# vovach777/llcomp

Measured on AMD Instinct MI355X. Metric: encode+decode MPix/s on 4K RGB8, bit-exact, higher is better.
Workload: dtype int32

## Files before the change

### llcomp_amd/csrc/codec.hip

```cpp
#include <hip/hip_runtime.h>

#include <algorithm>
#include <cstdlib>
#include <cstring>
#include <mutex>
#include <new>
#include <vector>

#include "../../include/llcomp_mi.h"
#include "codec_internal.hpp"
#include "container.hpp"
#include "geometry.hpp"
#include "kernels.hpp"
#include "resize.hpp"
#include "snapshot.hpp"
#include "tables.hpp"

using namespace llcomp_mi;

namespace llcomp_mi {

int status_from_bits(uint32_t bits) {
    if (bits & kStInternal) return LLCOMP_MI_HIP_ERROR;
    if (bits & kStBadExponent) return LLCOMP_MI_BAD_EXPONENT;
// ... 604 lines not shown
                    dev_alloc(reinterpret_cast<void**>(&k->d_scratch), b_scratch) == hipSuccess &&
                    dev_alloc(reinterpret_cast<void**>(&k->d_group_off), b_off) == hipSuccess &&
                    dev_alloc(reinterpret_cast<void**>(&k->d_total_tmp), 8) == hipSuccess &&
                    dev_alloc(reinterpret_cast<void**>(&k->d_counters), kCtrCount * 8) == hipSuccess &&
                    hipMemset(k->d_counters, 0, kCtrCount * 8) == hipSuccess;
    if (!ok) {
        llcomp_mi_codec_destroy(k);
        return LLCOMP_MI_NOMEM;
    }
    k->allocated_bytes = b_sym + b_lanes + b_scratch + b_off + 8;
    *out = k;
    return LLCOMP_MI_OK;
}

extern "C" {

void llcomp_mi_codec_destroy(llcomp_mi_codec* k) {
    llcomp_mi::codec_release(k);
}

int llcomp_mi_codec_prepare(llcomp_mi_codec* k, uint32_t what) {
    if (!k || (what & ~(LLCOMP_MI_PREPARE_ENCODE | LLCOMP_MI_PREPARE_DECODE | LLCOMP_MI_PREPARE_REGION | LLCOMP_MI_PREPARE_REGIONS |
                        LLCOMP_MI_PREPARE_RESIZED)))
        return LLCOMP_MI_BAD_ARGS;
    DeviceGuard guard(k->device);
    if (!guard.ok) return LLCOMP_MI_HIP_ERROR;
    if (what & LLCOMP_MI_PREPARE_ENCODE) {
        if (snapshot_mode(k->g)) {
            if (int rc = ensure_snapshot_arrays(k)) return rc;
        }
        if (!snapshot_mode(k->g) || snapshot_chunked(k->g))
            if (int rc = ensure_state_tables(k, k->need_states)) return rc;
    }
    if (what & LLCOMP_MI_PREPARE_DECODE)
        if (int rc = ensure_state_tables(k, k->need_states)) return rc;
    if (what & (LLCOMP_MI_PREPARE_REGION | LLCOMP_MI_PREPARE_REGIONS | LLCOMP_MI_PREPARE_RESIZED)) {
        if (int rc = ensure_region_arrays(k)) return rc;
        if (region_may_need_states(k))
            if (int rc = ensure_state_tables(k, true)) return rc;
    }
    if (what & LLCOMP_MI_PREPARE_REGIONS)
        if (int rc = ensure_regions_table(k)) return rc;
    if (what & LLCOMP_MI_PREPARE_RESIZED) {
        const uint64_t samples = uint64_t(k->g.frames) * k->g.w * k->g.h * k->g.c;
        if (int rc = ensure_regions_ring(k)) return rc;
        if (int rc = ensure_grown(k, k->d_box, k->box_cap, samples, samples)) return rc;
        if (int rc = ensure_grown(k, k->d_mid, k->mid_cap, samples, samples)) return rc;
    }
    return LLCOMP_MI_OK;
}

uint32_t llcomp_mi_codec_slices(const llcomp_mi_codec* k) { return k ? k->g.n_slices : 0; }
uint32_t llcomp_mi_codec_kernel_family(const llcomp_mi_codec* k) { return k ? (k->g.flags & 0xFFu) | (k->g.lane_shift << 8) | (k->g.lpw << 16) : 0; }
uint64_t llcomp_mi_codec_workspace_bytes(const llcomp_mi_codec* k) { return k ? k->workspace_bytes : 0; }
uint64_t llcomp_mi_codec_allocated_bytes(const llcomp_mi_codec* k) { return k ? k->allocated_bytes : 0; }
uint64_t llcomp_mi_codec_max_payload_bytes(const llcomp_mi_codec* k) {
    return k ? uint64_t(k->g.n_slices) * k->g.slice_cap : 0;
}

int llcomp_mi_codec_model(llcomp_mi_codec* k, const void* d_px, void* d_sym, void* stream) {
    if (!k || !d_px || !d_sym) return LLCOMP_MI_BAD_ARGS;
    DeviceGuard guard(k->device);
    if (!guard.ok) return LLCOMP_MI_HIP_ERROR;
    HIP_TRY(launch_model_fwd(k->g, static_cast<const uint8_t*>(d_px), static_cast<uint32_t*>(d_sym),
                             static_cast<hipStream_t>(stream)));
    return LLCOMP_MI_OK;
}

int llcomp_mi_codec_encode(llcomp_mi_codec* k, const void* d_px, void* d_payload, uint64_t payload_cap, void* d_slice_len,
                           void* d_total, void* d_status, void* stream) {
    if (!k || !d_px || !d_payload || !d_slice_len || !d_total || !d_status) return LLCOMP_MI_BAD_ARGS;
    DeviceGuard guard(k->device);
    if (!guard.ok) return LLCOMP_MI_HIP_ERROR;
    hipStream_t s = static_cast<hipStream_t>(stream);
    const Geometry& g = k->g;
    DoneGuard done_guard{k, s};
    HIP_TRY(hipMemsetAsync(d_status, 0, 4, s));
    if (!snapshot_mode(g) || snapshot_chunked(g)) {
        Timed t(k, s, 0);
        if (int rc = next_state_generation(k, s, k->need_states)) return rc;
    }
    {
        Timed t(k, s, 1);
        if (model_is_fused(g)) {
            HIP_TRY(launch_model_rows_fwd(g, static_cast<const uint8_t*>(d_px), static_cast<uint16_t*>(k->d_lane_order), s));
        } else {
            HIP_TRY(launch_model_fwd(g, static_cast<const uint8_t*>(d_px), static_cast<uint32_t*>(k->d_sym_or_rec), s));
            if (!snapshot_mode(g))
                HIP_TRY(launch_to_lane_order_u32(g, static_cast<const uint32_t*>(k->d_sym_or_rec),
                                                 static_cast<uint32_t*>(k->d_lane_order), s));
        }
    }
    if (snapshot_mode(g) && snapshot_chunked(g)) {
        if (int rc = ensure_snapshot_arrays(k)) return rc;
        const uint64_t gpat = state_generation_tag(k->state_generation);
        const uint32_t chunks = snapshot_chunks(g);
        hipStream_t ps = k->overlap ? k->aux : s;
        if (k->overlap) {
            HIP_TRY(hipEventRecord(k->ev_fork, s));
            HIP_TRY(hipStreamWaitEvent(k->aux, k->ev_fork, 0));
        }
        auto pass = [&](uint32_t c) -> int {
            Timed t(k, ps, 0);
            HIP_TRY(launch_snapshot_chunk(g, c, static_cast<const uint32_t*>(k->d_sym_or_rec), k->d_lane_order, k->d_snap_sorted, k->d_snap_banks,
                                          k->d_snap_res, k->d_snap_ctx, k->d_snap_io, k->d_states, gpat, ps));
            return LLCOMP_MI_OK;
        };
        auto coder = [&](uint32_t c) -> int {
            Timed t(k, s, 2);
            HIP_TRY(launch_encode_segment(g, k->d_snap_res, static_cast<uint64_t*>(k->d_snap_banks), k->d_scratch, static_cast<uint32_t*>(d_slice_len),
                                          static_cast<uint32_t*>(d_status), k->d_counters, c * kSnapMaxSamples, k->d_seg_state, s));
            return LLCOMP_MI_OK;
        };
        int rc = LLCOMP_MI_OK;
        if (k->overlap) {
            for (uint32_t c = 0; c < chunks && !rc; ++c) {
                rc = pass(c);
                if (!rc && hipEventRecord(k->ev_chunk[c], k->aux) != hipSuccess) rc = LLCOMP_MI_HIP_ERROR;
            }
            for (uint32_t c = 0; c < chunks; ++c) {
                if (hipStreamWaitEvent(s, k->ev_chunk[c], 0) != hipSuccess) { (void)hipGetLastError(); (void)hipStreamSynchronize(k->aux); }
                if (!rc) rc = coder(c);
            }
        } else {
            for (uint32_t c = 0; c < chunks && !rc; ++c) {
                rc = pass(c);
                if (!rc) rc = coder(c);
            }
        }
        if (rc) return rc;
    } else {
    if (snapshot_mode(g)) {
        if (int rc = ensure_snapshot_arrays(k)) return rc;
        Timed t(k, s, 0);
        HIP_TRY(launch_snapshot(g, static_cast<const uint32_t*>(k->d_sym_or_rec), k->d_lane_order, k->d_snap_sorted,
                                k->d_snap_banks, k->d_snap_res, s));
    }
    {
        Timed t(k, s, 2);
        const bool snap = snapshot_mode(g);
        HIP_TRY(launch_encode_slices(g, snap ? k->d_snap_res : k->d_lane_order, snap ? static_cast<uint64_t*>(k->d_snap_banks) : k->d_states,
                                     k->state_generation, k->d_scratch, static_cast<uint32_t*>(d_slice_len),
                                     k->d_group_off, static_cast<uint32_t*>(d_status), k->d_counters, s));
    }
    }
    {
        Timed t(k, s, 3);
        if (!encoder_writes_group_sums(g)) HIP_TRY(launch_group_sums(g, static_cast<const uint32_t*>(d_slice_len), k->d_group_off, s));
        HIP_TRY(launch_scan_groups(g, k->d_group_off, static_cast<uint64_t*>(d_total), s));
        HIP_TRY(launch_pack_payload(g, k->d_scratch, static_cast<const uint32_t*>(d_slice_len), k->d_group_off,
                                    static_cast<uint8_t*>(d_payload), payload_cap, static_cast<uint32_t*>(d_status), s));
    }
    ++k->n_encode;
    return LLCOMP_MI_OK;
}

int llcomp_mi_codec_decode(llcomp_mi_codec* k, const void* d_payload, uint64_t payload_bytes, const void* d_slice_len,
                           void* d_px, void* d_status, void* stream) {
    if (!k || !d_payload || !d_slice_len || !d_px || !d_status) return LLCOMP_MI_BAD_ARGS;
    DeviceGuard guard(k->device);
    if (!guard.ok) return LLCOMP_MI_HIP_ERROR;
    hipStream_t s = static_cast<hipStream_t>(stream);
    const Geometry& g = k->g;
    DoneGuard done_guard{k, s};
    HIP_TRY(hipMemsetAsync(d_status, 0, 4, s));
    {
        Timed t(k, s, 7);
        if (int rc = next_state_generation(k, s, k->need_states)) return rc;
    }
    {
        Timed t(k, s, 4);
        HIP_TRY(launch_group_sums(g, static_cast<const uint32_t*>(d_slice_len), k->d_group_off, s));
        HIP_TRY(launch_scan_groups(g, k->d_group_off, k->d_total_tmp, s));
    }
    {
        Timed t(k, s, 4);
        HIP_TRY(launch_stage_streams(g, static_cast<const uint8_t*>(d_payload), payload_bytes,
                                     static_cast<const uint32_t*>(d_slice_len), k->d_group_off, k->d_scratch,
                                     static_cast<uint32_t*>(d_status), s));
    }
    {
        Timed t(k, s, 5);
        const bool cache = use_bank_cache(k, g);
        HIP_TRY(launch_decode_slices(g, k->d_scratch, static_cast<const uint32_t*>(d_slice_len), k->d_states, k->state_generation,
                                     static_cast<int16_t*>(k->d_lane_order), static_cast<uint32_t*>(d_status), k->d_counters, cache, s));
        if (cache) queue_feedback(k, s);
    }
    {
        Timed t(k, s, 6);
        if (model_is_fused(g)) {
            HIP_TRY(launch_model_rows_inv(g, static_cast<const int16_t*>(k->d_lane_order), static_cast<uint8_t*>(d_px), s));
        } else {
            HIP_TRY(launch_from_lane_order_i16(g, static_cast<const int16_t*>(k->d_lane_order),
                                               static_cast<int16_t*>(k->d_sym_or_rec), s));
            HIP_TRY(launch_model_inv(g, static_cast<const int16_t*>(k->d_sym_or_rec), static_cast<uint8_t*>(d_px), s));
        }
    }
    ++k->n_decode;
    return LLCOMP_MI_OK;
}

uint32_t llcomp_mi_codec_region_family(const llcomp_mi_codec* k, uint32_t x, uint32_t y, uint32_t rw, uint32_t rh) {
    RegionBox box;
    Geometry sub;
    if (!k || region_setup(k, x, y, rw, rh, box, sub)) return 0;
    return (sub.flags & 0xFFu) | (sub.lane_shift << 8) | (sub.lpw << 16);
}

int llcomp_mi_codec_decode_region(llcomp_mi_codec* k, const void* d_payload, uint64_t payload_bytes, const void* d_slice_len, uint32_t x,
                                  uint32_t y, uint32_t rw, uint32_t rh, void* d_px, void* d_status, void* stream) {
    if (!k || !d_payload || !d_slice_len || !d_px || !d_status) return LLCOMP_MI_BAD_ARGS;
    RegionBox box;
    Geometry sub;
    if (int rc = region_setup(k, x, y, rw, rh, box, sub)) return rc;
    DeviceGuard guard(k->device);
    if (!guard.ok) return LLCOMP_MI_HIP_ERROR;
    if (int rc = ensure_region_arrays(k)) return rc;
    hipStream_t s = static_cast<hipStream_t>(stream);
    const Geometry& g = k->g;
    DoneGuard done_guard{k, s};
    HIP_TRY(hipMemsetAsync(d_status, 0, 4, s));
    {
        Timed t(k, s, 7);
        if (int rc = next_state_generation(k, s, slices_need_state_tables(sub))) return rc;
// ... 298 lines not shown
```

### llcomp_amd/csrc/geometry.hpp

```cpp
#pragma once
#include <algorithm>
#include <cstdint>
#include <cstdlib>

#if defined(__HIPCC__)
#define LLMI_HD __host__ __device__
#else
#define LLMI_HD
#endif

namespace llcomp_mi {

constexpr uint32_t kMaxChannels = 255;

struct Geometry {
    uint32_t frames, w, h, c;
    uint32_t tile_w, tile_h, planar;
    uint32_t ntx, nty;
    uint32_t slices_per_frame;
    uint32_t n_slices;
    uint32_t slice_cap;
    uint32_t nch;
    uint32_t lane_shift;
    uint32_t slice_samples;
    uint32_t lpw;
    uint32_t flags;
};
enum : uint32_t {
    kGeoRows = 1u,
    kGeoLdsTable = 2u,
    kGeoForceReplay = 4u,
    kGeoSmallModel = 8u,
    kGeoSnapshot = 16u,
    kGeoBankCache = 32u,
};
constexpr uint32_t kSnapMaxSamples = 4096;
constexpr uint32_t kSnapMaxChunks = 4;

struct Tuning {
    int lane_shift = -1;
    int lpw = 0;
    bool norows = false;
    bool noldstab = false;
    bool force_replay = false;
    bool nosnap = false;
    bool nocache = false;
    int overlap = 2;
    bool nofeedback = false;
};
inline Tuning tuning_from_env() {
    Tuning t;
    auto num = [](const char* name, long lo, long hi, int dflt) {
        const char* e = std::getenv(name);
        if (!e || !*e) return dflt;
        const long v = std::strtol(e, nullptr, 10);
        return (v >= lo && v <= hi) ? int(v) : dflt;
    };
    auto flag = [](const char* name) { const char* e = std::getenv(name); return e && e[0] == '1'; };
    t.lane_shift = num("LLCOMP_MI_LANE_SHIFT", 0, 6, -1);
    t.lpw = num("LLCOMP_MI_LPW", 1, 64, 0);
    t.norows = flag("LLCOMP_MI_NOROWS");
    t.noldstab = flag("LLCOMP_MI_NOLDSTAB");
    t.force_replay = flag("LLCOMP_MI_FORCE_REPLAY");
    t.nosnap = flag("LLCOMP_MI_NOSNAP");
    t.nocache = flag("LLCOMP_MI_NOCACHE");
    t.nofeedback = flag("LLCOMP_MI_NOFEEDBACK");
    t.overlap = num("LLCOMP_MI_OVERLAP", 0, 2, 2);
    return t;
}

LLMI_HD inline uint32_t snapshot_chunks(const Geometry& g) { return (g.slice_samples + kSnapMaxSamples - 1) / kSnapMaxSamples; }
LLMI_HD inline uint32_t snapshot_cap(const Geometry& g) {
    return g.slice_samples <= kSnapMaxSamples ? (g.slice_samples + 15u) & ~15u : snapshot_chunks(g) * kSnapMaxSamples;
}

constexpr int kBankCacheLog2 = 5;
inline int bank_cache_log2(const Geometry& g) { return (g.flags & kGeoBankCache) ? kBankCacheLog2 : 0; }

LLMI_HD inline size_t lane_order_index(const Geometry& g, uint32_t id, uint32_t k) {
    const uint32_t gw = 1u << g.lane_shift;
    return ((size_t(id >> g.lane_shift) * g.slice_samples + k) << g.lane_shift) + (id & (gw - 1));
}

struct SliceRect {
    uint32_t frame, x0, y0, sw, sh, ch;
};

LLMI_HD inline SliceRect slice_rect(const Geometry& g, uint32_t id) {
    SliceRect r;
    r.frame = id / g.slices_per_frame;
    uint32_t s = id - r.frame * g.slices_per_frame;
    uint32_t tile = s;
    r.ch = 0;
    if (g.planar) {
        tile = s / g.c;
        r.ch = s - tile * g.c;
    }
    const uint32_t ty = tile / g.ntx, tx = tile - ty * g.ntx;
    r.x0 = tx * g.tile_w;
    r.y0 = ty * g.tile_h;
    r.sw = g.w - r.x0 < g.tile_w ? g.w - r.x0 : g.tile_w;
    r.sh = g.h - r.y0 < g.tile_h ? g.h - r.y0 : g.tile_h;
    return r;
}

inline uint32_t default_lane_shift(uint32_t n_slices) {
    constexpr uint32_t kMinWaves = 96;
    uint32_t s = 6;
    while (s > 0 && (n_slices >> s) < kMinWaves) --s;
    return s;
}

inline bool make_geometry(Geometry& g, uint32_t frames, uint32_t w, uint32_t h, uint32_t c, uint32_t tile_w,
                          uint32_t tile_h, uint32_t planar, const Tuning& tune = Tuning{}, bool small_model = false) {
    if (!frames || !w || !h || c < 1 || c > kMaxChannels) return false;
    if (tile_w == 0 || tile_w > w) tile_w = w;
    if (tile_h == 0 || tile_h > h) tile_h = h;
    const uint64_t samples = uint64_t(w) * h * c;
    if (samples >= (1ull << 31)) return false;
    g.frames = frames; g.w = w; g.h = h; g.c = c;
    g.tile_w = tile_w; g.tile_h = tile_h; g.planar = planar ? 1 : 0;
    g.ntx = (w + tile_w - 1) / tile_w;
    g.nty = (h + tile_h - 1) / tile_h;
    const uint64_t spf = uint64_t(g.ntx) * g.nty * (g.planar ? c : 1);
    if (spf * frames >= (1ull << 31)) return false;
    g.slices_per_frame = uint32_t(spf);
    g.n_slices = uint32_t(spf * frames);
    g.nch = g.planar ? 1 : c;
    const uint64_t cap = (uint64_t(tile_w) * tile_h * g.nch * 13 + 32 + 15) & ~15ull;
    g.slice_cap = uint32_t(cap < 0x7FFFFFF0ull ? cap : 0x7FFFFFF0ull);
    g.slice_samples = tile_w * tile_h * g.nch;
    g.lane_shift = tune.lane_shift >= 0 ? uint32_t(tune.lane_shift) : default_lane_shift(g.n_slices);
    if (tune.lane_shift < 0 && g.tile_h > 1 && g.slice_samples > kSnapMaxSamples && g.n_slices <= 512) g.lane_shift = 0;
    const uint32_t gw = 1u << g.lane_shift;
    g.lpw = gw;
    if (tune.lpw >= 1) {
        uint32_t p = 1;
        while (p * 2 <= uint32_t(tune.lpw) && p * 2 <= gw) p *= 2;
        g.lpw = p;
    }
    g.flags = 0;
    if (g.tile_h == 1 && !tune.norows && g.nch <= 4) g.flags |= kGeoRows;
    else if (g.lpw == 1 && !tune.noldstab) g.flags |= kGeoLdsTable;
    else if (g.slice_samples <= kSnapMaxSamples * kSnapMaxChunks && !tune.nosnap) g.flags |= kGeoSnapshot;
    if (!(g.flags & (kGeoRows | kGeoLdsTable)) && g.nch <= 4 && !tune.nocache) g.flags |= kGeoBankCache;
    if (tune.force_replay) g.flags |= kGeoForceReplay;
    if (small_model) g.flags |= kGeoSmallModel;
    return true;
}

inline uint64_t legacy_read_bound(uint64_t samples) { return 65 * samples + 2; }
inline void fit_legacy_stream(Geometry& g, uint64_t bytes) {
    const uint64_t cap = (bytes + 16 + 15) & ~15ull;
    if (cap > g.slice_cap) g.slice_cap = uint32_t(cap < 0x7FFFFFF0ull ? cap : 0x7FFFFFF0ull);
}

struct RegionBox {
    uint32_t tx0, ty0, tx1, ty1;
};
inline bool region_box(uint32_t w, uint32_t h, uint32_t tile_w, uint32_t tile_h, uint32_t x, uint32_t y, uint32_t rw, uint32_t rh,
// ... 85 lines not shown
```

### llcomp_amd/csrc/kernels.hpp

```cpp
#pragma once
#include <hip/hip_runtime.h>

#include <cstdint>

#include "geometry.hpp"

namespace llcomp_mi {

enum : uint32_t { kStOverflow = 1u, kStBadExponent = 2u, kStTruncated = 4u, kStInternal = 8u  };

enum : uint32_t {
    kCtrDecCachedWaves = 0,
    kCtrDecBypassedWaves = 1,
    kCtrCacheLookups = 2,
    kCtrCacheMisses = 3,
    kCtrCacheWritebacks = 4,
    kCtrDecReplays = 5,
    kCtrEncCarryBacks = 6,
    kCtrGenerationWraps = 7,
    kCtrDecLaunchesCached = 8,
    kCtrDecLaunchesPlainByFeedback = 9,
    kCtrCount = 16,
};

hipError_t launch_model_fwd(const Geometry& g, const uint8_t* d_px, uint32_t* d_sym, hipStream_t stream);
hipError_t launch_model_inv(const Geometry& g, const int16_t* d_rec, uint8_t* d_px, hipStream_t stream);

uint32_t lane_groups(const Geometry& g);
uint32_t slice_capacity_samples(const Geometry& g);
hipError_t launch_to_lane_order_u32(const Geometry& g, const uint32_t* d_img, uint32_t* d_lanes, hipStream_t stream);
hipError_t launch_from_lane_order_i16(const Geometry& g, const int16_t* d_lanes, int16_t* d_img, hipStream_t stream);

bool model_is_fused(const Geometry& g);
hipError_t launch_model_rows_fwd(const Geometry& g, const uint8_t* d_px, uint16_t* d_lanes, hipStream_t stream);
hipError_t launch_model_rows_inv(const Geometry& g, const int16_t* d_lanes, uint8_t* d_px, hipStream_t stream);

bool rows_mode(const Geometry& g);
bool slices_need_state_tables(const Geometry& g);

hipError_t launch_encode_slices(const Geometry& g, const void* d_sym, uint64_t* d_states, uint32_t generation, uint8_t* d_scratch,
                                uint32_t* d_slice_len, uint64_t* d_group_off, uint32_t* d_status, unsigned long long* d_counters,
                                hipStream_t stream);
uint64_t state_generation_tag(uint32_t generation);
hipError_t launch_encode_segment(const Geometry& g, const void* d_res, uint64_t* d_banks, uint8_t* d_scratch, uint32_t* d_slice_len,
                                 uint32_t* d_status, unsigned long long* d_counters, uint32_t seg_first, uint32_t* d_seg_state,
                                 hipStream_t stream);
bool encoder_writes_group_sums(const Geometry& g);
hipError_t launch_group_sums(const Geometry& g, const uint32_t* d_slice_len, uint64_t* d_group_off, hipStream_t stream);
hipError_t launch_scan_groups(const Geometry& g, uint64_t* d_group_off, uint64_t* d_total, hipStream_t stream);
hipError_t launch_frame_bytes(const Geometry& g, const uint32_t* d_slice_len, uint64_t* d_frame_bytes, hipStream_t stream);
hipError_t launch_pack_payload(const Geometry& g, const uint8_t* d_units, const uint32_t* d_slice_len,
                               const uint64_t* d_group_off, uint8_t* d_payload, uint64_t payload_cap,
                               uint32_t* d_status, hipStream_t stream);
hipError_t launch_stage_streams(const Geometry& g, const uint8_t* d_payload, uint64_t payload_bytes,
                                const uint32_t* d_slice_len, const uint64_t* d_group_off, uint8_t* d_units,
                                uint32_t* d_status, hipStream_t stream);
hipError_t launch_copy_segments(const uint8_t* d_src, uint8_t* d_dst, const uint64_t* d_src_off, const uint64_t* d_dst_off,
                                const uint64_t* d_len, uint32_t n_seg, uint64_t max_len, hipStream_t stream);
hipError_t launch_range_sums(const uint32_t* d_vals, const uint64_t* d_start, const uint64_t* d_count, uint64_t* d_out, uint32_t n,
                             uint32_t cap, hipStream_t stream);
hipError_t launch_decode_slices(const Geometry& g, const uint8_t* d_units, const uint32_t* d_slice_len,
                                uint64_t* d_states, uint32_t generation, int16_t* d_rec, uint32_t* d_status, unsigned long long* d_counters,
                                bool bank_cache, hipStream_t stream);

hipError_t launch_region_index(const Geometry& full, const Geometry& sub, const RegionBox& box, const uint32_t* d_slice_len,
                               const uint64_t* d_group_off, uint32_t* d_sub_len, uint64_t* d_sub_off, hipStream_t stream);
hipError_t launch_stage_region_streams(const Geometry& sub, const uint8_t* d_payload, uint64_t payload_bytes, const uint32_t* d_sub_len,
                                       const uint64_t* d_sub_off, uint8_t* d_units, uint32_t* d_status, hipStream_t stream);
struct Crop {
    uint32_t x0, y0, rw, rh;
};
hipError_t launch_model_inv_crop(const Geometry& sub, const int16_t* d_rec, uint8_t* d_px, const Crop& cr, hipStream_t stream);
hipError_t launch_model_rows_inv_crop(const Geometry& sub, const int16_t* d_lanes, uint8_t* d_px, const Crop& cr, hipStream_t stream);

hipError_t launch_regions_index(const Geometry& full, const Geometry& sub, const RegionsFrame* d_tab, const uint32_t* d_slice_len,
                                const uint64_t* d_group_off, uint32_t* d_sub_len, uint64_t* d_sub_off, hipStream_t stream);
hipError_t launch_model_inv_crops(const Geometry& sub, const int16_t* d_rec, uint8_t* d_px, const RegionsFrame* d_tab, uint32_t rw,
                                  uint32_t rh, hipStream_t stream);
hipError_t launch_model_rows_inv_crops(const Geometry& sub, const int16_t* d_lanes, uint8_t* d_px, const RegionsFrame* d_tab, uint32_t rw,
                                       uint32_t rh, hipStream_t stream);

}
```

### llcomp_amd/csrc/model_kernels.hip

```cpp
#include <algorithm>

#include "device_common.hpp"
#include "kernels.hpp"

namespace llcomp_mi {

namespace {

constexpr int kMW = 256;
constexpr int kMH = 32;

template <int C>
__device__ __forceinline__ void rct_forward(const uint8_t* p, int16_t (&o)[C]) {
    if constexpr (C >= 3) {
        const int g = p[1], cb = int(p[2]) - g, cr = int(p[0]) - g;
        o[0] = int16_t(cr);
        o[1] = int16_t(g + (cb + cr) / 4);
        o[2] = int16_t(cb);
        if constexpr (C == 4) o[3] = p[3];
    } else {
#pragma unroll
        for (int k = 0; k < C; ++k) o[k] = p[k];
    }
}
// ... 1062 lines not shown
    const uint32_t q4 = threadIdx.x & 15;
    for (uint32_t tt = threadIdx.x >> 4; tt < ntiles; tt += 16) {
        const uint32_t sw = tiles[tt].khi, klo = tiles[tt].klo, kb = k0 + 4 * q4;
        if (kb >= sw || kb + 4 <= klo) continue;
        uint8_t bytes[4 * C];
#pragma unroll
        for (int i = 0; i < 4; ++i) {
            const int16_t* s = &tile[4 * q4 + i][col0 + tt * C];
            if constexpr (C >= 3) {
                int r = s[0], gg = s[1], bb = s[2];
                gg -= (r + bb) / 4;
                r += gg;
                bb += gg;
                bytes[i * C + 0] = uint8_t(min(max(r, 0), 255));
                bytes[i * C + 1] = uint8_t(min(max(gg, 0), 255));
                bytes[i * C + 2] = uint8_t(min(max(bb, 0), 255));
                if constexpr (C == 4) bytes[i * C + 3] = uint8_t(s[3]);
            } else {
#pragma unroll
                for (int c = 0; c < C; ++c) bytes[i * C + c] = uint8_t(s[c]);
            }
        }
        const uint32_t npx = sw - kb < 4 ? sw - kb : 4;
        if (npx < 4 || kb < klo) {
            for (uint32_t i = kb < klo ? klo - kb : 0u; i < npx; ++i)
                for (uint32_t c = 0; c < uint32_t(C); ++c) px[tiles[tt].base + (long long)(kb + i) * C + c] = bytes[i * C + c];
            continue;
        }
        uint32_t w[C];
#pragma unroll
        for (int c = 0; c < C; ++c)
            w[c] = uint32_t(bytes[4 * c]) | (uint32_t(bytes[4 * c + 1]) << 8) | (uint32_t(bytes[4 * c + 2]) << 16) |
                   (uint32_t(bytes[4 * c + 3]) << 24);
        __builtin_memcpy(px + tiles[tt].base + size_t(kb) * C, w, 4 * C);
    }
}


}

#define LLMI_DISPATCH_C(c, CALL) \
    switch (c) {                 \
        case 1: { constexpr int C = 1; CALL; } break; \
        case 2: { constexpr int C = 2; CALL; } break; \
        case 3: { constexpr int C = 3; CALL; } break; \
        case 4: { constexpr int C = 4; CALL; } break; \
        default: return hipErrorInvalidValue; \
    }

hipError_t launch_model_fwd(const Geometry& g, const uint8_t* d_px, uint32_t* d_sym, hipStream_t stream) {
    if (g.c > 4) {
        const size_t npix = size_t(g.frames) * g.h * g.w;
        k_model_fwd_any<<<dim3(uint32_t((npix + 255) / 256)), dim3(256), 0, stream>>>(g, d_px, d_sym, npix);
        return hipGetLastError();
    }
    const uint32_t nbx = (g.w + kMW - 1) / kMW;
    const uint32_t spt = (g.tile_h + kMH - 1) / kMH;
    const uint64_t blocks = uint64_t(nbx) * spt * g.nty * g.frames;
    if (blocks == 0 || blocks > 0x7FFFFFFFull) return hipErrorInvalidValue;
    LLMI_DISPATCH_C(g.c, (k_model_fwd<C><<<dim3(uint32_t(blocks)), dim3(kMW), 0, stream>>>(g, d_px, d_sym)));
    return hipGetLastError();
}

uint32_t lane_groups(const Geometry& g) { return (g.n_slices + (1u << g.lane_shift) - 1) >> g.lane_shift; }
uint32_t slice_capacity_samples(const Geometry& g) { return g.slice_samples; }

hipError_t launch_to_lane_order_u32(const Geometry& g, const uint32_t* d_img, uint32_t* d_lanes, hipStream_t stream) {
    const uint32_t max_n = slice_capacity_samples(g);
    const uint64_t blocks = uint64_t(lane_groups(g)) * ((max_n + 63) / 64);
    if (blocks == 0 || blocks > 0x7FFFFFFFull) return hipErrorInvalidValue;
    k_to_lane_order<uint32_t><<<dim3(uint32_t(blocks)), dim3(256), 0, stream>>>(g, max_n, d_img, d_lanes);
    return hipGetLastError();
}

hipError_t launch_from_lane_order_i16(const Geometry& g, const int16_t* d_lanes, int16_t* d_img, hipStream_t stream) {
    const uint32_t max_n = slice_capacity_samples(g);
    const uint64_t blocks = uint64_t(lane_groups(g)) * ((max_n + 63) / 64);
    if (blocks == 0 || blocks > 0x7FFFFFFFull) return hipErrorInvalidValue;
    k_from_lane_order<int16_t><<<dim3(uint32_t(blocks)), dim3(256), 0, stream>>>(g, max_n, d_lanes, d_img);
    return hipGetLastError();
}

bool model_is_fused(const Geometry& g) { return g.planar && rows_mode(g) && g.c <= 4; }

hipError_t launch_model_rows_fwd(const Geometry& g, const uint8_t* d_px, uint16_t* d_lanes, hipStream_t stream) {
    const uint64_t blocks = xcd_grid(lane_groups(g), (g.tile_w + 63) / 64);
    if (blocks == 0 || blocks > 0x7FFFFFFFull) return hipErrorInvalidValue;
    LLMI_DISPATCH_C(g.c, (k_model_rows_fwd<C><<<dim3(uint32_t(blocks)), dim3(256), 0, stream>>>(g, d_px, d_lanes)));
    return hipGetLastError();
}

hipError_t launch_model_rows_inv(const Geometry& g, const int16_t* d_lanes, uint8_t* d_px, hipStream_t stream) {
    const uint64_t blocks = xcd_chunk_grid(lane_groups(g), (g.tile_w + 63) / 64);
    if (blocks == 0 || blocks > 0x7FFFFFFFull) return hipErrorInvalidValue;
    LLMI_DISPATCH_C(g.c, (k_model_rows_inv<C><<<dim3(uint32_t(blocks)), dim3(256), 0, stream>>>(g, d_lanes, d_px)));
    return hipGetLastError();
}

hipError_t launch_model_inv(const Geometry& g, const int16_t* d_rec, uint8_t* d_px, hipStream_t stream) {
    const size_t npix = size_t(g.frames) * g.h * g.w;
    if (g.c > 4) {
        k_model_inv_any<<<dim3(uint32_t((npix + 255) / 256)), dim3(256), 0, stream>>>(g, d_rec, d_px, npix);
        return hipGetLastError();
    }
    const uint32_t blocks = uint32_t(std::min<size_t>((npix + 255) / 256, 256 * 16));
    LLMI_DISPATCH_C(g.c, (k_model_inv<C><<<dim3(blocks), dim3(256), 0, stream>>>(g, d_rec, d_px, npix)));
    return hipGetLastError();
}

hipError_t launch_group_sums(const Geometry& g, const uint32_t* d_slice_len, uint64_t* d_group_off, hipStream_t stream) {
    k_group_sums<<<dim3((g.n_slices + kSumThreads - 1) / kSumThreads), dim3(kSumThreads), 0, stream>>>(d_slice_len, g.n_slices, g.lane_shift, d_group_off);
    return hipGetLastError();
}

hipError_t launch_frame_bytes(const Geometry& g, const uint32_t* d_slice_len, uint64_t* d_frame_bytes, hipStream_t stream) {
    k_frame_bytes<<<dim3(g.frames), dim3(256), 0, stream>>>(d_slice_len, g.slices_per_frame, d_frame_bytes);
    return hipGetLastError();
}

hipError_t launch_scan_groups(const Geometry& g, uint64_t* d_group_off, uint64_t* d_total, hipStream_t stream) {
    k_scan_groups<<<dim3(1), dim3(kScanThreads), 0, stream>>>(d_group_off, lane_groups(g), d_total);
    return hipGetLastError();
}

hipError_t launch_copy_segments(const uint8_t* d_src, uint8_t* d_dst, const uint64_t* d_src_off, const uint64_t* d_dst_off,
                                const uint64_t* d_len, uint32_t n_seg, uint64_t max_len, hipStream_t stream) {
    if (n_seg == 0) return hipSuccess;
    if (n_seg > 65535) return hipErrorInvalidValue;
    const uint64_t pieces = (max_len / 4 + kSegPieceDwords - 1) / kSegPieceDwords;
    const uint32_t gx = uint32_t(std::min<uint64_t>(std::max<uint64_t>(pieces, 1), 1024));
    k_copy_segments<<<dim3(gx, n_seg), dim3(256), 0, stream>>>(d_src, d_dst, d_src_off, d_dst_off, d_len);
    return hipGetLastError();
}

hipError_t launch_range_sums(const uint32_t* d_vals, const uint64_t* d_start, const uint64_t* d_count, uint64_t* d_out, uint32_t n,
                             uint32_t cap, hipStream_t stream) {
    if (!n) return hipSuccess;
    k_range_sums<<<dim3(n), dim3(256), 0, stream>>>(d_vals, d_start, d_count, d_out, cap);
    return hipGetLastError();
}

hipError_t launch_pack_payload(const Geometry& g, const uint8_t* d_units, const uint32_t* d_slice_len,
                               const uint64_t* d_offsets, uint8_t* d_payload, uint64_t payload_cap,
                               uint32_t* d_status, hipStream_t stream) {
    k_pack_payload<<<dim3(lane_groups(g)), dim3(256), 0, stream>>>(g, reinterpret_cast<const uint4*>(d_units), d_slice_len,
                                                                   d_offsets, d_payload, payload_cap, d_status);
    return hipGetLastError();
}

hipError_t launch_region_index(const Geometry& full, const Geometry& sub, const RegionBox& box, const uint32_t* d_slice_len,
                               const uint64_t* d_group_off, uint32_t* d_sub_len, uint64_t* d_sub_off, hipStream_t stream) {
    if (sub.n_slices == 0) return hipErrorInvalidValue;
    k_region_index<<<dim3((sub.n_slices + 255) / 256), dim3(256), 0, stream>>>(full, sub, box, d_slice_len, d_group_off, d_sub_len, d_sub_off);
    return hipGetLastError();
}

hipError_t launch_stage_region_streams(const Geometry& sub, const uint8_t* d_payload, uint64_t payload_bytes, const uint32_t* d_sub_len,
                                       const uint64_t* d_sub_off, uint8_t* d_units, uint32_t* d_status, hipStream_t stream) {
    k_stage_region_streams<<<dim3(lane_groups(sub)), dim3(256), 0, stream>>>(sub, d_payload, payload_bytes, d_sub_len, d_sub_off,
                                                                             reinterpret_cast<uint4*>(d_units), d_status);
    return hipGetLastError();
}

hipError_t launch_model_inv_crop(const Geometry& sub, const int16_t* d_rec, uint8_t* d_px, const Crop& cr, hipStream_t stream) {
    const size_t npix = size_t(sub.frames) * cr.rh * cr.rw;
    if (npix == 0 || uint64_t(cr.x0) + cr.rw > sub.w || uint64_t(cr.y0) + cr.rh > sub.h) return hipErrorInvalidValue;
// ... 60 lines not shown
```

### llcomp_amd/csrc/slice_kernels.hip

```cpp
#include <algorithm>

#include "device_common.hpp"
#include "kernels.hpp"

#ifndef LLMI_ASM_ENC
#define LLMI_ASM_ENC 1
#endif
#if LLMI_ASM_ENC
#include "enc_rows_asm.hpp"
#endif
#ifndef LLMI_ASM_DEC
#define LLMI_ASM_DEC 1
#endif
#if LLMI_ASM_DEC
#include "dec_rows_asm.hpp"
#endif

namespace llcomp_mi {

namespace {

#ifdef LLMI_CLOCK_PROBE
constexpr uint32_t kProbeSlots = 1u << 15;
__device__ unsigned long long g_probe[2][kProbeSlots][2];
// ... 411 lines not shown
            return *reinterpret_cast<const uint2*>(gbank + size_t(i >> 3) * (2 * row) + ((i & 7u) << 3) + 2 * lofs);
        };
        uint32_t i = 0, end = total;
        [[maybe_unused]] uint32_t* const rec = SEG ? seg_state + size_t(id) * 16 : nullptr;
        if constexpr (SEG) {
            if (seg_first >= total) return;
            i = seg_first;
            end = min(total, seg_first + kSnapMaxSamples);
            if (seg_first) {
                const uint4 a = *reinterpret_cast<const uint4*>(rec), b = *reinterpret_cast<const uint4*>(rec + 4);
                const uint4 s0 = *reinterpret_cast<const uint4*>(rec + 8), s1 = *reinterpret_cast<const uint4*>(rec + 12);
                e.low = a.x; e.range = a.y; e.wp = e.base + a.z; e.flushed = int32_t(a.w);
                e.carries = b.x; hot = b.y != 0;
                e.oofs += (uint32_t(e.flushed) >> 4) * e.ostep;
                uint32_t* const st = reinterpret_cast<uint32_t*>(e.area);
                st[0] = s0.x; st[1] = s0.y; st[2] = s0.z; st[3] = s0.w; st[4] = s1.x; st[5] = s1.y; st[6] = s1.z; st[7] = s1.w;
            }
        }
#if LLMI_ASM_ENC
        EncRowsExtra xs{0u, 0u, 0u};
        unsigned long long low_range = e.low | ((unsigned long long)e.range << 32);
#endif
        auto code = [&](int res, uint2 bk) {
#if LLMI_ASM_ENC
            enc_snap_sample_asm(low_range, e.wp, xs, bk.x, bk.y, res, e.base);
            if (__builtin_expect(xs.any_pend != 0, 0)) {
                xs.any_pend = 0;
                if (xs.pend) enc_carry_back_flushed(e);
                xs.pend = 0;
            }
#else
            Bank bank{{bk.x, bk.y}, nullptr};
            if (hot) enc_residual<true, false>(e, bank, tab, res); else enc_residual<false, false>(e, bank, tab, res);
            hot = __builtin_amdgcn_readfirstlane(2 * __popcll(__ballot(res != 0)) >= __popcll(__ballot(true)));
#endif
        };
        const uint32_t todo = end - i, todo0 = __builtin_amdgcn_readfirstlane(todo);
        const bool same = __builtin_amdgcn_ballot_w64(todo != todo0) == 0;
        const uint32_t n_bulk = i + (same ? todo0 & ~3u : 0);
        int r0 = load_res(i), r1 = load_res(i + 1), r2 = load_res(i + 2), r3 = load_res(i + 3);
        uint2 b0 = load_bank(i), b1 = load_bank(i + 1), b2 = load_bank(i + 2), b3 = load_bank(i + 3);
#define LLMI_SNAP_SAMPLE(R, B, AHEAD)                          \
        {                                                          \
            const int rc = int(consume_here(uint32_t(R)));        \
            uint2 bc = B;                                          \
            bc.x = consume_here(bc.x);                             \
            R = load_res(i + AHEAD);                               \
            B = load_bank(i + AHEAD);                              \
            if (e.wp >= e.base + 16) enc_flush16(e);               \
            code(rc, bc);                                          \
        }
        for (; i < n_bulk; i += 4) {
            LLMI_SNAP_SAMPLE(r0, b0, 4)
            LLMI_SNAP_SAMPLE(r1, b1, 5)
            LLMI_SNAP_SAMPLE(r2, b2, 6)
            LLMI_SNAP_SAMPLE(r3, b3, 7)
        }
        for (; i < end; ++i) {
            LLMI_SNAP_SAMPLE(r0, b0, 4)
            {
                const int tr = r0;
                const uint2 tb = b0;
                r0 = r1; r1 = r2; r2 = r3; r3 = tr;
                b0 = b1; b1 = b2; b2 = b3; b3 = tb;
            }
        }
#undef LLMI_SNAP_SAMPLE
#if LLMI_ASM_ENC
        e.low = uint32_t(low_range);
        e.range = uint32_t(low_range >> 32);
#endif
        if constexpr (SEG) {
            if (end < total) {
                const uint32_t* const st = reinterpret_cast<const uint32_t*>(e.area);
                *reinterpret_cast<uint4*>(rec) = make_uint4(e.low, e.range, e.wp - e.base, uint32_t(e.flushed));
                *reinterpret_cast<uint4*>(rec + 4) = make_uint4(e.carries, hot ? 1u : 0u, 0u, 0u);
                *reinterpret_cast<uint4*>(rec + 8) = make_uint4(st[0], st[1], st[2], st[3]);
                *reinterpret_cast<uint4*>(rec + 12) = make_uint4(st[4], st[5], st[6], st[7]);
                return;
            }
        }
    } else if constexpr (ROWS) {
        for (uint32_t k = 0; k < 6; ++k) rowbank[k * 64 + threadIdx.x] = 0;
        const uint32_t grp = __builtin_amdgcn_readfirstlane(id >> g.lane_shift);
        const char* const gsym = reinterpret_cast<const char*>(sym + ((size_t(grp) * g.slice_samples) << g.lane_shift));
        uint32_t sofs = (id & ((1u << g.lane_shift) - 1)) * uint32_t(sizeof(SYM)), sstep = uint32_t(sizeof(SYM)) << g.lane_shift;
        asm volatile("" : "+v"(sstep));
        auto load_sym = [&](uint32_t ofs) -> uint32_t { return *reinterpret_cast<const SYM*>(gsym + ofs); };
        uint32_t s0 = load_sym(sofs);
        sofs += sstep;
        uint32_t s1 = total > 1 ? load_sym(sofs) : 0;
        sofs += sstep;
        uint32_t bank_base = uint32_t(uintptr_t((lds_u8_ptr) reinterpret_cast<uint8_t*>(rowbank))) + threadIdx.x * 4;
        asm volatile("" : "+v"(bank_base));
#if LLMI_ASM_ENC
        EncRowsExtra xs{0u, 0u, 0u};
        unsigned long long low_range = e.low | ((unsigned long long)e.range << 32);
#endif
        auto code = [&](uint32_t sy) {
            uint32_t bofs;
            int res;
            if constexpr (sizeof(SYM) == 2) {
                bofs = (sy >> 3) & 0x600u;
                res = int(sy << 20) >> 20;
            } else {
                bofs = (((sy & 0xFFFF) * 109u) >> 7) & 0x600u;
                res = int(sy) >> 16;
            }
#if LLMI_ASM_ENC
            enc_rows_sample_asm(low_range, e.wp, xs, bank_base + bofs, res, e.base);
            if (__builtin_expect(xs.any_pend != 0, 0)) {
                xs.any_pend = 0;
                if (xs.pend) enc_carry_back_flushed(e);
                xs.pend = 0;
            }
#else
            uint32_t* bp = reinterpret_cast<uint32_t*>(reinterpret_cast<uint8_t*>(rowbank) + threadIdx.x * 4 + bofs);
            Bank bank{{bp[0], bp[64]}, reinterpret_cast<uint8_t*>(bp)};
            if (hot) enc_residual<true, true>(e, bank, tab, res); else enc_residual<false, true>(e, bank, tab, res);
            hot = __builtin_amdgcn_readfirstlane(2 * __popcll(__ballot(res != 0)) >= __popcll(__ballot(true)));
#endif
        };
        const uint32_t total0 = __builtin_amdgcn_readfirstlane(total);
        const bool same = __builtin_amdgcn_ballot_w64(total != total0) == 0;
        const uint32_t n_bulk = same && total0 > 2 ? total0 - 2 : 0;
        uint32_t i = 0;
        for (; i < n_bulk; ++i) {
            s0 = consume_here(s0);
            const uint32_t s2 = load_sym(sofs);
            sofs += sstep;
            if (e.wp >= e.base + 16) enc_flush16(e);
            code(s0);
            s0 = s1;
            s1 = s2;
        }
        for (; i < total; ++i) {
            s0 = consume_here(s0);
            const uint32_t s2 = i + 2 < total ? load_sym(sofs) : 0;
            sofs += sstep;
            if (e.wp >= e.base + 16) enc_flush16(e);
            code(s0);
            s0 = s1;
            s1 = s2;
        }
#if LLMI_ASM_ENC
        e.low = uint32_t(low_range);
        e.range = uint32_t(low_range >> 32);
#endif
    } else {
        uint64_t* banks;
        uint32_t bsh;
        if constexpr (LDSTAB) {
            banks = reinterpret_cast<uint64_t*>(dyn_lds);
            bsh = 0;
        } else {
            banks = states + ((size_t(id >> g.lane_shift) * kContexts) << g.lane_shift) + (id & ((1u << g.lane_shift) - 1));
            bsh = g.lane_shift;
        }
        uint32_t fk = 0;
        auto fetch = [&]() -> uint32_t { return p0[size_t(fk++) * GW]; };
        uint32_t s0 = fetch();
        uint32_t s1 = total > 1 ? fetch() : 0;
        uint64_t b0 = bank_fresh<LDSTAB>(banks[size_t(s0 & 0xFFFF) << bsh], gpat);
        for (uint32_t i = 0; i < total; ++i) {
            const uint32_t s2 = i + 2 < total ? fetch() : 0;
            const uint32_t ctx0 = s0 & 0xFFFF, ctx1 = s1 & 0xFFFF;
            const int res = int(s0) >> 16;
            uint64_t raw1 = (i + 1 < total) ? banks[size_t(ctx1) << bsh] : 0;
            Bank bank{{uint32_t(b0), uint32_t(b0 >> 32)}, nullptr};
            if (hot) enc_residual<true, false>(e, bank, tab, res); else enc_residual<false, false>(e, bank, tab, res);
            hot = __builtin_amdgcn_readfirstlane(2 * __popcll(__ballot(res != 0)) >= __popcll(__ballot(true)));
            b0 = uint64_t(bank.w[0]) | (uint64_t(bank.w[1]) << 32);
            if constexpr (!LDSTAB) drain_vector_memory();
            uint64_t b1 = bank_fresh<LDSTAB>(raw1, gpat);
            banks[size_t(ctx0) << bsh] = bank_tagged<LDSTAB>(b0, gpat);
            if (ctx1 == ctx0) b1 = b0;
            b0 = b1;
            if (e.wp >= e.base + 16) enc_flush16(e);
            s0 = s1;
            s1 = s2;
        }
    }
    int32_t n_bytes = enc_pos(e);
    enc_finish_and_count(e, n_bytes);
    LLMI_PROBE_STOP(0);
    if (n_bytes > e.cap) {
        atomicOr(status, kStOverflow);
        n_bytes = e.cap;
    }
    slice_len[id] = uint32_t(n_bytes);
    publish_count(counters, kCtrEncCarryBacks, e.carries);
    if (group_sum) {
        unsigned long long live = __ballot(1), sum = 0;
        while (live) {
            const int lane = __builtin_ctzll(live);
            sum += uint32_t(__builtin_amdgcn_readlane(n_bytes, lane));
            live &= live - 1;
        }
        if (threadIdx.x == 0) group_sum[blockIdx.x] = sum;
    }
}

template <int SLOT, bool INLDS>
__device__ __forceinline__ void dec_put_state(Bank& b, uint32_t half) {
    if constexpr (INLDS) *reinterpret_cast<uint16_t*>(b.lds + widebank_byte(SLOT)) = uint16_t(half >> 16);
    else set_slot_state<SLOT>(b.w, half & 0xFF);
}
template <int SLOT, bool INLDS>
__device__ __forceinline__ entry_t dec_entry(const Bank& b, const entry_t* tab) {
    if constexpr (INLDS) return lds_entry(wide_offset<SLOT>(b.w));
    else return tab[slot_state<SLOT>(b.w)];
}
template <bool INLDS>
__device__ __forceinline__ void dec_fetch_slot0(Entries& E, const Bank& b, const entry_t* tab) { E.e0 = dec_entry<0, INLDS>(b, tab); }
template <bool INLDS>
__device__ __forceinline__ void dec_fetch_rest(Entries& E, const Bank& b, const entry_t* tab) {
    E.e1 = dec_entry<1, INLDS>(b, tab);
    E.e2 = dec_entry<2, INLDS>(b, tab);
    E.e3 = dec_entry<3, INLDS>(b, tab);
    E.e4 = dec_entry<4, INLDS>(b, tab);
    E.e5 = dec_entry<5, INLDS>(b, tab);
    E.e6 = dec_entry<6, INLDS>(b, tab);
    E.e7 = dec_entry<7, INLDS>(b, tab);
}
// ... 461 lines not shown
                if (gave_up) atomicAdd(counters + kCtrDecBypassedWaves, 1ull);
            }
        }
        publish_count(counters, kCtrDecReplays, d.replays);
        }
    }
    LLMI_PROBE_STOP(1);
}

}

#ifdef LLMI_CLOCK_PROBE
extern "C" uint32_t llcomp_mi_probe_read(unsigned long long* out) {
    if (out) {
        (void)hipDeviceSynchronize();
        (void)hipMemcpyFromSymbol(out, HIP_SYMBOL(g_probe), sizeof(g_probe));
        static unsigned long long zeros[2][kProbeSlots][2];
        (void)hipMemcpyToSymbol(HIP_SYMBOL(g_probe), zeros, sizeof(g_probe));
    }
    return kProbeSlots;
}
extern "C" void llcomp_mi_probe_read_parts(unsigned long long* out) {
    (void)hipDeviceSynchronize();
    (void)hipMemcpyFromSymbol(out, HIP_SYMBOL(g_probe_parts), sizeof(g_probe_parts));
}
#endif

#define LLMI_DISPATCH_SLICE(nch, rows, lds, ...)                                                             \
    switch (((nch) > 4 ? 0 : (nch)) * 4 + ((rows) ? 2 : 0) + ((lds) ? 1 : 0)) {                               \
        case 0: { constexpr int C = 0; constexpr bool R = false; constexpr bool T = false; __VA_ARGS__; } break;    \
        case 1: { constexpr int C = 0; constexpr bool R = false; constexpr bool T = true; __VA_ARGS__; } break;     \
        case 4: { constexpr int C = 1; constexpr bool R = false; constexpr bool T = false; __VA_ARGS__; } break;    \
        case 5: { constexpr int C = 1; constexpr bool R = false; constexpr bool T = true; __VA_ARGS__; } break;     \
        case 6: { constexpr int C = 1; constexpr bool R = true; constexpr bool T = false; __VA_ARGS__; } break;     \
        case 8: { constexpr int C = 2; constexpr bool R = false; constexpr bool T = false; __VA_ARGS__; } break;    \
        case 9: { constexpr int C = 2; constexpr bool R = false; constexpr bool T = true; __VA_ARGS__; } break;     \
        case 10: { constexpr int C = 2; constexpr bool R = true; constexpr bool T = false; __VA_ARGS__; } break;    \
        case 12: { constexpr int C = 3; constexpr bool R = false; constexpr bool T = false; __VA_ARGS__; } break;   \
        case 13: { constexpr int C = 3; constexpr bool R = false; constexpr bool T = true; __VA_ARGS__; } break;    \
        case 14: { constexpr int C = 3; constexpr bool R = true; constexpr bool T = false; __VA_ARGS__; } break;    \
        case 16: { constexpr int C = 4; constexpr bool R = false; constexpr bool T = false; __VA_ARGS__; } break;   \
        case 17: { constexpr int C = 4; constexpr bool R = false; constexpr bool T = true; __VA_ARGS__; } break;    \
        case 18: { constexpr int C = 4; constexpr bool R = true; constexpr bool T = false; __VA_ARGS__; } break;    \
        default: return hipErrorInvalidValue;                                                               \
    }

bool rows_mode(const Geometry& g) { return (g.flags & kGeoRows) != 0; }
static bool states_in_lds(const Geometry& g) { return (g.flags & kGeoLdsTable) != 0; }
bool slices_need_state_tables(const Geometry& g) { return !rows_mode(g) && !states_in_lds(g); }

constexpr size_t kLdsTableBytes = size_t(kContexts) * 8;
template <typename K>
hipError_t allow_big_lds(K kernel) {
    return hipFuncSetAttribute(reinterpret_cast<const void*>(kernel), hipFuncAttributeMaxDynamicSharedMemorySize,
                               int(kLdsTableBytes));
}

static bool coder_in_segments(const Geometry& g) { return (g.flags & kGeoSnapshot) != 0 && snapshot_chunks(g) > 1; }
bool encoder_writes_group_sums(const Geometry& g) { return g.lpw == (1u << g.lane_shift) && !coder_in_segments(g); }

hipError_t launch_encode_segment(const Geometry& g, const void* d_res, uint64_t* d_banks, uint8_t* d_scratch, uint32_t* d_slice_len,
                                 uint32_t* d_status, unsigned long long* d_counters, uint32_t seg_first, uint32_t* d_seg_state,
                                 hipStream_t stream) {
    if (!coder_in_segments(g) || !d_seg_state) return hipErrorInvalidValue;
    const uint32_t blocks = (g.n_slices + g.lpw - 1) / g.lpw;
    k_encode_slices<0, false, uint32_t, false, true, true><<<dim3(blocks), dim3(64), LLMI_ASM_ENC ? kRowsEncLdsBytes : 0, stream>>>(
        g, g.lpw, static_cast<const uint32_t*>(d_res), d_banks, d_scratch, d_slice_len, nullptr, d_status, 0, d_counters, seg_first, d_seg_state);
    return hipGetLastError();
}

uint64_t state_generation_tag(uint32_t generation) {
    uint64_t t = 0;
    for (int i = 0; i < 8; ++i) t |= uint64_t((generation >> i) & 1u) << (8 * i + 7);
    return t;
}

hipError_t launch_encode_slices(const Geometry& g, const void* d_sym, uint64_t* d_states, uint32_t generation, uint8_t* d_scratch,
                                uint32_t* d_slice_len, uint64_t* d_group_off, uint32_t* d_status, unsigned long long* d_counters,
                                hipStream_t stream) {
    const uint64_t gpat = slices_need_state_tables(g) ? state_generation_tag(generation) : 0;
    const uint32_t lpw = g.lpw;
    const uint32_t blocks = (g.n_slices + lpw - 1) / lpw;
    uint64_t* const d_group_sum = encoder_writes_group_sums(g) ? d_group_off : nullptr;
    if (model_is_fused(g)) {
        k_encode_slices<1, true, uint16_t><<<dim3(blocks), dim3(64), LLMI_ASM_ENC ? kRowsEncLdsBytes : 0, stream>>>(
            g, lpw, static_cast<const uint16_t*>(d_sym), d_states, d_scratch, d_slice_len, d_group_sum, d_status, gpat, d_counters);
        return hipGetLastError();
    }
    if (g.flags & kGeoSnapshot) {
        k_encode_slices<0, false, uint32_t, false, true><<<dim3(blocks), dim3(64), LLMI_ASM_ENC ? kRowsEncLdsBytes : 0, stream>>>(
            g, lpw, static_cast<const uint32_t*>(d_sym), d_states, d_scratch, d_slice_len, d_group_sum, d_status, 0, d_counters);
        return hipGetLastError();
    }
    const bool lds = states_in_lds(g);
    LLMI_DISPATCH_SLICE(g.nch, rows_mode(g), lds, {
        auto kernel = k_encode_slices<C, R, uint32_t, T>;
        if (T) {
            const hipError_t e = allow_big_lds(kernel);
            if (e != hipSuccess) return e;
        }
        kernel<<<dim3(blocks), dim3(64), T ? kLdsTableBytes : (R && LLMI_ASM_ENC ? kRowsEncLdsBytes : 0), stream>>>(
            g, lpw, static_cast<const uint32_t*>(d_sym), d_states, d_scratch, d_slice_len, d_group_sum, d_status, gpat, d_counters, 0u, nullptr);
    });
    return hipGetLastError();
}

hipError_t launch_decode_slices(const Geometry& g, const uint8_t* d_units, const uint32_t* d_slice_len,
                                uint64_t* d_states, uint32_t generation, int16_t* d_rec, uint32_t* d_status, unsigned long long* d_counters,
                                bool bank_cache, hipStream_t stream) {
    const uint64_t gpat = slices_need_state_tables(g) ? state_generation_tag(generation) : 0;
    const uint32_t lpw = g.lpw;
    const uint32_t blocks = (g.n_slices + lpw - 1) / lpw;
    const uint32_t arg = lpw | ((g.flags & kGeoForceReplay) ? 0x100u : 0u);
    const bool lds = states_in_lds(g);
    if (bank_cache_log2(g) == kBankCacheLog2 && bank_cache) {
#define LLMI_DECODE_CACHED(NCHV)                                                                                          \
    k_decode_slices<NCHV, false, false, kBankCacheLog2><<<dim3(blocks), dim3(64), bank_cache_lds_bytes(kBankCacheLog2), stream>>>( \
        g, arg, d_units, d_slice_len, d_states, d_rec, d_status, gpat, d_counters)
        switch (g.nch) {
            case 1: LLMI_DECODE_CACHED(1); break;
            case 2: LLMI_DECODE_CACHED(2); break;
            case 3: LLMI_DECODE_CACHED(3); break;
            case 4: LLMI_DECODE_CACHED(4); break;
            default: return hipErrorInvalidValue;
        }
#undef LLMI_DECODE_CACHED
        return hipGetLastError();
    }
    LLMI_DISPATCH_SLICE(g.nch, rows_mode(g), lds, {
        auto kernel = k_decode_slices<C, R, T>;
        if (T) {
            const hipError_t e = allow_big_lds(kernel);
            if (e != hipSuccess) return e;
        }
        kernel<<<dim3(blocks), dim3(64), T ? kLdsTableBytes : 0, stream>>>(g, arg, d_units, d_slice_len, d_states,
                                                                          d_rec, d_status, gpat, d_counters);
    });
    return hipGetLastError();
}

}
```

Before: 26930.

## Fuse forward model into rows encoder reading pixels directly

In fused rows mode the encoder kernel now reads raw interleaved pixels and computes the colour transform, prediction residual and context bank inside the coding loop. The separate model_rows_fwd kernel and its uint16 lane-order intermediate buffer are skipped. This removes one kernel launch and a full write and read of the intermediate residual array. In exchange the encoder does more ALU work per symbol and issues unaligned, strided pixel loads, with byte-wise loads near the end of the buffer.

After: 28760 (median of 6 runs). 1.07x the previous value.

```diff
diff --git a/llcomp_amd/csrc/codec.hip b/llcomp_amd/csrc/codec.hip
--- a/llcomp_amd/csrc/codec.hip
+++ b/llcomp_amd/csrc/codec.hip
@@ -710,7 +710,8 @@
     }
     {
         Timed t(k, s, 1);
-        if (model_is_fused(g)) {
+        if (rows_encoder_reads_pixels(g)) {
+        } else if (model_is_fused(g)) {
             HIP_TRY(launch_model_rows_fwd(g, static_cast<const uint8_t*>(d_px), static_cast<uint16_t*>(k->d_lane_order), s));
         } else {
             HIP_TRY(launch_model_fwd(g, static_cast<const uint8_t*>(d_px), static_cast<uint32_t*>(k->d_sym_or_rec), s));
@@ -767,7 +768,8 @@
     {
         Timed t(k, s, 2);
         const bool snap = snapshot_mode(g);
-        HIP_TRY(launch_encode_slices(g, snap ? k->d_snap_res : k->d_lane_order, snap ? static_cast<uint64_t*>(k->d_snap_banks) : k->d_states,
+        const void* in = snap ? k->d_snap_res : rows_encoder_reads_pixels(g) ? d_px : k->d_lane_order;
+        HIP_TRY(launch_encode_slices(g, in, snap ? static_cast<uint64_t*>(k->d_snap_banks) : k->d_states,
                                      k->state_generation, k->d_scratch, static_cast<uint32_t*>(d_slice_len),
                                      k->d_group_off, static_cast<uint32_t*>(d_status), k->d_counters, s));
     }
diff --git a/llcomp_amd/csrc/geometry.hpp b/llcomp_amd/csrc/geometry.hpp
--- a/llcomp_amd/csrc/geometry.hpp
+++ b/llcomp_amd/csrc/geometry.hpp
@@ -76,6 +76,13 @@
 
 constexpr int kBankCacheLog2 = 5;
 inline int bank_cache_log2(const Geometry& g) { return (g.flags & kGeoBankCache) ? kBankCacheLog2 : 0; }
+
+LLMI_HD inline uint32_t rows_px_dwords(uint64_t tile_base, uint32_t samples, uint32_t c, uint64_t batch_bytes) {
+    if (tile_base + 4 > batch_bytes) return 0;
+    const uint64_t k = (batch_bytes - 4 - tile_base) / c + 1;
+    return k < samples ? uint32_t(k) : samples;
+}
+LLMI_HD inline uint32_t rows_px_tail(uint32_t c) { return 1 + (4 + c - 1) / c; }
 
 LLMI_HD inline size_t lane_order_index(const Geometry& g, uint32_t id, uint32_t k) {
     const uint32_t gw = 1u << g.lane_shift;
diff --git a/llcomp_amd/csrc/kernels.hpp b/llcomp_amd/csrc/kernels.hpp
--- a/llcomp_amd/csrc/kernels.hpp
+++ b/llcomp_amd/csrc/kernels.hpp
@@ -32,6 +32,7 @@
 hipError_t launch_from_lane_order_i16(const Geometry& g, const int16_t* d_lanes, int16_t* d_img, hipStream_t stream);
 
 bool model_is_fused(const Geometry& g);
+bool rows_encoder_reads_pixels(const Geometry& g);
 hipError_t launch_model_rows_fwd(const Geometry& g, const uint8_t* d_px, uint16_t* d_lanes, hipStream_t stream);
 hipError_t launch_model_rows_inv(const Geometry& g, const int16_t* d_lanes, uint8_t* d_px, hipStream_t stream);
 
diff --git a/llcomp_amd/csrc/model_kernels.hip b/llcomp_amd/csrc/model_kernels.hip
--- a/llcomp_amd/csrc/model_kernels.hip
+++ b/llcomp_amd/csrc/model_kernels.hip
@@ -1168,6 +1168,9 @@
 }
 
 bool model_is_fused(const Geometry& g) { return g.planar && rows_mode(g) && g.c <= 4; }
+bool rows_encoder_reads_pixels(const Geometry& g) {
+    return model_is_fused(g) && (uint64_t(63 / g.c + 2) * g.tile_w * g.c + 4 < (1ull << 31));
+}
 
 hipError_t launch_model_rows_fwd(const Geometry& g, const uint8_t* d_px, uint16_t* d_lanes, hipStream_t stream) {
     const uint64_t blocks = xcd_grid(lane_groups(g), (g.tile_w + 63) / 64);
diff --git a/llcomp_amd/csrc/slice_kernels.hip b/llcomp_amd/csrc/slice_kernels.hip
--- a/llcomp_amd/csrc/slice_kernels.hip
+++ b/llcomp_amd/csrc/slice_kernels.hip
@@ -517,14 +517,59 @@
         }
     } else if constexpr (ROWS) {
         for (uint32_t k = 0; k < 6; ++k) rowbank[k * 64 + threadIdx.x] = 0;
-        const uint32_t grp = __builtin_amdgcn_readfirstlane(id >> g.lane_shift);
-        const char* const gsym = reinterpret_cast<const char*>(sym + ((size_t(grp) * g.slice_samples) << g.lane_shift));
-        uint32_t sofs = (id & ((1u << g.lane_shift) - 1)) * uint32_t(sizeof(SYM)), sstep = uint32_t(sizeof(SYM)) << g.lane_shift;
+        constexpr bool PX = sizeof(SYM) == 1;
+        const char* gsym;
+        uint32_t sofs, sstep;
+        [[maybe_unused]] uint32_t n_dword = total;
+        [[maybe_unused]] uint32_t psh = 0, msub = 0, my = 0, large = 0;
+        [[maybe_unused]] int pl = 128, pL = 128;
+        if constexpr (PX) {
+            const uint32_t C = g.c;
+            const unsigned long long tbase = ((unsigned long long)(r.frame) * g.h + r.y0) * g.w * C + (unsigned long long)(r.x0) * C;
+            const unsigned long long wbase = (unsigned long long)uint32_t(__builtin_amdgcn_readfirstlane(uint32_t(tbase))) |
+                                             ((unsigned long long)uint32_t(__builtin_amdgcn_readfirstlane(uint32_t(tbase >> 32))) << 32);
+            gsym = reinterpret_cast<const char*>(sym) + wbase;
+            sofs = uint32_t(tbase - wbase);
+            sstep = C;
+            const unsigned long long total_bytes = (unsigned long long)(g.frames) * g.h * g.w * C;
+            n_dword = rows_px_dwords(tbase, total, C, total_bytes);
+            psh = 8 * r.ch;
+            msub = C >= 3 && (r.ch == 0 || r.ch == 2) ? ~0u : 0u;
+            my = C >= 3 && r.ch == 1 ? ~0u : 0u;
+            large = (g.flags & kGeoSmallModel) ? 0u : ~0u;
+            asm volatile("" : "+v"(psh), "+v"(msub), "+v"(my));
+        } else {
+            const uint32_t grp = __builtin_amdgcn_readfirstlane(id >> g.lane_shift);
+            gsym = reinterpret_cast<const char*>(sym + ((size_t(grp) * g.slice_samples) << g.lane_shift));
+            sofs = (id & ((1u << g.lane_shift) - 1)) * uint32_t(sizeof(SYM));
+            sstep = uint32_t(sizeof(SYM)) << g.lane_shift;
+        }
         asm volatile("" : "+v"(sstep));
-        auto load_sym = [&](uint32_t ofs) -> uint32_t { return *reinterpret_cast<const SYM*>(gsym + ofs); };
-        uint32_t s0 = load_sym(sofs);
+        auto load_sym = [&](uint32_t ofs) -> uint32_t {
+            if constexpr (PX) {
+                uint32_t w;
+                __builtin_memcpy(&w, gsym + ofs, 4);
+                return w;
+            } else {
+                return *reinterpret_cast<const SYM*>(gsym + ofs);
+            }
+        };
+        auto load_at = [&](uint32_t ofs, uint32_t k) -> uint32_t {
+            if constexpr (PX) {
+                if (k >= n_dword) {
+                    const uint8_t* p = reinterpret_cast<const uint8_t*>(gsym + ofs);
+                    uint32_t w = p[0];
+                    if (g.c > 1) w |= uint32_t(p[1]) << 8;
+                    if (g.c > 2) w |= uint32_t(p[2]) << 16;
+                    if (g.c > 3) w |= uint32_t(p[3]) << 24;
+                    return w;
+                }
+            }
+            return load_sym(ofs);
+        };
+        uint32_t s0 = load_at(sofs, 0);
         sofs += sstep;
-        uint32_t s1 = total > 1 ? load_sym(sofs) : 0;
+        uint32_t s1 = total > 1 ? load_at(sofs, 1) : 0;
         sofs += sstep;
         uint32_t bank_base = uint32_t(uintptr_t((lds_u8_ptr) reinterpret_cast<uint8_t*>(rowbank))) + threadIdx.x * 4;
         asm volatile("" : "+v"(bank_base));
@@ -532,10 +577,22 @@
         EncRowsExtra xs{0u, 0u, 0u};
         unsigned long long low_range = e.low | ((unsigned long long)e.range << 32);
 #endif
-        auto code = [&](uint32_t sy) {
+        auto code = [&](uint32_t sy, uint32_t i) {
             uint32_t bofs;
             int res;
-            if constexpr (sizeof(SYM) == 2) {
+            if constexpr (PX) {
+                const uint32_t G = (sy >> 8) & 0xFF;
+                const int sum = int(sy & 0xFF) + int((sy >> 16) & 0xFF) - 2 * int(G);
+                const int t = (sum + int((uint32_t(sum) >> 31) * 3u)) >> 2;
+                const int v = int(__builtin_amdgcn_ubfe(sy, psh, 8)) - int(G & msub) + (t & int(my));
+                const int dq = (pL - pl) & int(i >= 2 ? large : 0u);
+                const int sg = dq >> 31;
+                const uint32_t aq = uint32_t((dq ^ sg) - sg);
+                bofs = ((aq + 511u) & 0x200u) + ((aq + 508u) & 0x200u);
+                res = ((v - pl) ^ sg) - sg;
+                pL = pl;
+                pl = v;
+            } else if constexpr (sizeof(SYM) == 2) {
                 bofs = (sy >> 3) & 0x600u;
                 res = int(sy << 20) >> 20;
             } else {
@@ -558,23 +615,24 @@
         };
         const uint32_t total0 = __builtin_amdgcn_readfirstlane(total);
         const bool same = __builtin_amdgcn_ballot_w64(total != total0) == 0;
-        const uint32_t n_bulk = same && total0 > 2 ? total0 - 2 : 0;
+        const uint32_t tail = PX ? rows_px_tail(g.c) : 2u;
+        const uint32_t n_bulk = same && total0 > tail ? total0 - tail : 0;
         uint32_t i = 0;
         for (; i < n_bulk; ++i) {
             s0 = consume_here(s0);
             const uint32_t s2 = load_sym(sofs);
             sofs += sstep;
             if (e.wp >= e.base + 16) enc_flush16(e);
-            code(s0);
+            code(s0, i);
             s0 = s1;
             s1 = s2;
         }
         for (; i < total; ++i) {
             s0 = consume_here(s0);
-            const uint32_t s2 = i + 2 < total ? load_sym(sofs) : 0;
+            const uint32_t s2 = i + 2 < total ? load_at(sofs, i + 2) : 0;
             sofs += sstep;
             if (e.wp >= e.base + 16) enc_flush16(e);
-            code(s0);
+            code(s0, i);
             s0 = s1;
             s1 = s2;
         }
@@ -1202,6 +1260,11 @@
     const uint32_t lpw = g.lpw;
     const uint32_t blocks = (g.n_slices + lpw - 1) / lpw;
     uint64_t* const d_group_sum = encoder_writes_group_sums(g) ? d_group_off : nullptr;
+    if (rows_encoder_reads_pixels(g)) {
+        k_encode_slices<1, true, uint8_t><<<dim3(blocks), dim3(64), LLMI_ASM_ENC ? kRowsEncLdsBytes : 0, stream>>>(
+            g, lpw, static_cast<const uint8_t*>(d_sym), d_states, d_scratch, d_slice_len, d_group_sum, d_status, gpat, d_counters);
+        return hipGetLastError();
+    }
     if (model_is_fused(g)) {
         k_encode_slices<1, true, uint16_t><<<dim3(blocks), dim3(64), LLMI_ASM_ENC ? kRowsEncLdsBytes : 0, stream>>>(
             g, lpw, static_cast<const uint16_t*>(d_sym), d_states, d_scratch, d_slice_len, d_group_sum, d_status, gpat, d_counters);
```
